# chenhonghua/MVIP-NeRF

Measured on NVIDIA B200. Metric: rays/sec (train fwd+bwd, 64+64 samples), higher is better.
Workload: dtype bf16

## Files before the change

mvip_nerf_b200/csrc/mlp_backward.cu:

```cuda
#include "mlp_pair.cuh"
#include <stdlib.h>

namespace {
using namespace mlp;

constexpr int kCSteps = 9;

struct ChainParams {
  const uint8_t* packed;
  const float4* d_raw;
  const uint8_t* stash;
  uint8_t* dz;
  int64_t n_points;
  int64_t n_tiles;
  uint32_t* flags;
  uint32_t* cons_stamp;
  uint32_t* next_pair;
  uint32_t* credit;
  int throttle_units;
  int throttle_cycles;
  int throttle_gain;
  int stagger;
};
constexpr int kFlagsPerTile = 10;

__device__ __forceinline__ int chain_nchunks(int s) { return s == 0 ? 2 : 4; }

constexpr int kStagePts = 64;
constexpr int kSubStages = kTile / kStagePts;
constexpr uint32_t kHalf = kStagePts * 128;
constexpr int kNumItems = 11;
constexpr size_t kPartialSlotBytes = (size_t)256 * 320 * sizeof(float);
constexpr int kFusedSlots = 80;

#ifndef MVIP_PROF_CLUSTER
#define MVIP_PROF_CLUSTER 0
#endif
__device__ unsigned long long g_wprof[8];
__device__ unsigned long long g_lag[80][4];
__device__ __forceinline__ uint32_t globaltimer_lo() {
  uint32_t t;
  asm volatile("mov.u32 %0, %%globaltimer_lo;" : "=r"(t));
  return t;
}
#ifdef MVIP_TRACE_BWD
__device__ long long g_btrace[20][12];
#define BTR(hs, ev) do { if (tr_on) g_btrace[hs][ev] = clock64(); } while (0)
#else
#define BTR(hs, ev)
#endif

struct WItem {
  int a_chunk;
  int m_blocks;
  int nb;
  int b_chunk[5];
  int dst;
  int ld;
  int col[5];
  int valid[5];
  int bias;
  int cost;
};

__constant__ WItem kItems[kNumItems] = {
    {kDzHidden, 1, 5, {33, 34, 35, 36, 37}, kPViewsW, 283, {0, 64, 128, 192, 256}, {64, 64, 64, 64, 27}, kPViewsB, 7},
    {kDzFeat, 2, 4, {29, 30, 31, 32, 0}, kPFeatW, 256, {0, 64, 128, 192, 0}, {64, 64, 64, 64, 0}, kPFeatB, 8},
    {kDzTrunk + 0, 2, 4, {25, 26, 27, 28, 0}, 14, 256, {0, 64, 128, 192, 0}, {64, 64, 64, 64, 0}, 15, 8},
    {kDzTrunk + 4, 2, 4, {21, 22, 23, 24, 0}, 12, 256, {0, 64, 128, 192, 0}, {64, 64, 64, 64, 0}, 13, 8},
    {kDzTrunk + 8, 2, 4, {17, 18, 19, 20, 0}, 10, 319, {63, 127, 191, 255, 0}, {64, 64, 64, 64, 0}, 11, 8},
    {kDzTrunk + 8, 2, 1, {0, 0, 0, 0, 0}, 10, 319, {0, 0, 0, 0, 0}, {63, 0, 0, 0, 0}, -1, 5},
    {kDzTrunk + 12, 2, 4, {13, 14, 15, 16, 0}, 8, 256, {0, 64, 128, 192, 0}, {64, 64, 64, 64, 0}, 9, 8},
    {kDzTrunk + 16, 2, 4, {9, 10, 11, 12, 0}, 6, 256, {0, 64, 128, 192, 0}, {64, 64, 64, 64, 0}, 7, 8},
    {kDzTrunk + 20, 2, 4, {5, 6, 7, 8, 0}, 4, 256, {0, 64, 128, 192, 0}, {64, 64, 64, 64, 0}, 5, 8},
    {kDzTrunk + 24, 2, 4, {1, 2, 3, 4, 0}, 2, 256, {0, 64, 128, 192, 0}, {64, 64, 64, 64, 0}, 3, 8},
    {kDzTrunk + 28, 2, 1, {0, 0, 0, 0, 0}, 0, 63, {0, 0, 0, 0, 0}, {63, 0, 0, 0, 0}, 1, 5},
};
constexpr int kRealItems = kNumItems;

struct Segment {
  int item;
  int t0, t1;
  int stride;
};

struct WParams {
  const uint8_t* stash;
  const uint8_t* dz;
  int64_t n_tiles;
  float* partials;
  float* bias_partials;
  Segment* segs;
};

constexpr int kFThreads = 512;
constexpr int kFSlots = 8, kFLag = 2;
constexpr int kFStages = (4 * 64) / kStagePts;
constexpr uint32_t kFStageBytes = 4 * kHalf;
constexpr uint32_t kFSmemW = 0;
constexpr uint32_t kFSmemStg = kFSmemW + kFSlots * kSlotBytes2;
constexpr uint32_t kFSmemWg = kFSmemStg + 2 * kActChunk;
constexpr uint32_t kFSmemBytes = kFSmemWg + kFStages * kFStageBytes;
struct FItem {
  int slot_item;
  int flag;
  int a_src, b_src;
  int a_chunk[2][2];
  int b_chunk[2][2];
  int n_b, n_mma;
  int transposed;
  int ld, col0, n_cols;
  int drain_ranks;
  int bias_ranks;
  int zero_lo, zero_hi;
  int cost;
};
constexpr int kFusedItems = 12;
#ifndef MVIP_SMALL_COST
#define MVIP_SMALL_COST 10
#endif
#define MVIP_FULL_ITEM(it, fl, a0, b0) {it, fl, 0, 1, {{a0, a0 + 1}, {a0 + 2, a0 + 3}}, {{b0, b0 + 1}, {b0 + 2, b0 + 3}}, 2, 256, 0, 256, 0, 256, 3, 3, 0, 0, 10}
__constant__ FItem kFItems[kFusedItems] = {
    MVIP_FULL_ITEM(1, 1, kDzFeat, 29),
    MVIP_FULL_ITEM(2, 2, kDzTrunk + 0, 25),
    MVIP_FULL_ITEM(3, 3, kDzTrunk + 4, 21),
    MVIP_FULL_ITEM(4, 4, kDzTrunk + 8, 17),
    MVIP_FULL_ITEM(6, 5, kDzTrunk + 12, 13),
    MVIP_FULL_ITEM(7, 6, kDzTrunk + 16, 9),
    MVIP_FULL_ITEM(8, 7, kDzTrunk + 20, 5),
    MVIP_FULL_ITEM(9, 8, kDzTrunk + 24, 1),
    {5, 4, 0, 1, {{kDzTrunk + 8, kDzTrunk + 9}, {kDzTrunk + 10, kDzTrunk + 11}}, {{0, 0}, {0, 0}}, 1, 128, 0, 64, 0, 64, 3, 0, 0, 0, MVIP_SMALL_COST},
    {10, 9, 0, 1, {{kDzTrunk + 28, kDzTrunk + 29}, {kDzTrunk + 30, kDzTrunk + 31}}, {{0, 0}, {0, 0}}, 1, 128, 0, 64, 0, 64, 3, 3, 0, 0, MVIP_SMALL_COST},
    {0, 0, 1, 0, {{33, 34}, {35, 36}}, {{kDzHidden, 0}, {kDzHidden + 1, 0}}, 1, 128, 1, 320, 0, 128, 3, 0, 256, 320, MVIP_SMALL_COST},
    {0, 0, 0, 1, {{kDzHidden, kDzHidden + 1}, {kDzHidden, kDzHidden + 1}}, {{37, 0}, {37, 0}}, 1, 128, 0, 320, 256, 64, 1, 1, 0, 256, MVIP_SMALL_COST},
};
struct FusedPlan {
  unsigned char item[kFusedSlots], k[kFusedSlots], n[kFusedSlots];
};


__global__ void __cluster_dims__(2, 1, 1) __launch_bounds__(kFThreads, 1)
backward_fused_kernel(const ChainParams p, const WParams wp, const FusedPlan plan) {
  constexpr int kG = kGroupBars2;
  extern __shared__ uint8_t smem_raw[];
  uint8_t* smem = reinterpret_cast<uint8_t*>((reinterpret_cast<uintptr_t>(smem_raw) + 1023) & ~uintptr_t(1023));
  __shared__ uint64_t bar_gfull[kG], bar_gempty[kG], bar_acc, bar_act, bar_hi;
  __shared__ uint64_t bar_wfull[kFStages], bar_wempty[kFStages], bar_wacc;
  __shared__ uint64_t bar_sfull[2], bar_sfree[2];
  __shared__ uint32_t tmem_base_s;
  __shared__ uint32_t it_q[4];
  __shared__ uint64_t bar_it[4];
  __shared__ uint32_t w_ready_s;
  volatile uint32_t* w_ready = &w_ready_s;

  const int tid = threadIdx.x, warp = tid >> 5, lane = tid & 31;
  const uint32_t rank = cluster_ctarank();
  const int cluster = blockIdx.x >> 1, n_clusters = gridDim.x >> 1;
  const int64_t n_pairs = (p.n_tiles + 1) / 2;
  const uint8_t* wT = p.packed + kFwdBytes;

  const int wj = plan.item[cluster], wk = plan.k[cluster], wn = plan.n[cluster];
  const FItem& fit = kFItems[wj];
  const bool w_active = wk < p.n_tiles;
  auto watch_flags = [&]() {
    if (!w_active) return;
    const int n_my = ((int)p.n_tiles - wk + wn - 1) / wn;
    unsigned long long l_sum = 0, l_max = 0;
    int ready = 0;
    while (ready < n_my) {
      const int idx = ready + lane;
      uint32_t stamp = 0;
      if (idx < n_my) stamp = ld_acquire_gpu(p.flags + (size_t)(wk + idx * wn) * kFlagsPerTile + fit.flag);
      const uint32_t got = __ballot_sync(0xffffffffu, stamp != 0u);
      const int prefix = (got == 0xffffffffu) ? 32 : __ffs(~got) - 1;
      if (prefix > 0) {
        if (lane < prefix) { const uint32_t lag = globaltimer_lo() - (stamp & ~1u); l_sum += lag; l_max = lag > l_max ? lag : l_max; }
        ready += prefix;
        __threadfence_block();
        if (lane == 0) *w_ready = (uint32_t)ready;
      } else {
        __nanosleep(100);
      }
    }
    for (int o = 16; o > 0; o >>= 1) {
      l_sum += __shfl_xor_sync(0xffffffffu, l_sum, o);
      const unsigned long long m = __shfl_xor_sync(0xffffffffu, l_max, o);
      l_max = m > l_max ? m : l_max;
    }
    if (rank == 0 && lane == 0) { g_lag[cluster][0] = l_sum; g_lag[cluster][1] = l_max; }
  };

  if (tid == 0) {
    for (int i = 0; i < kG; ++i) {
      mbar_init(&bar_gfull[i], rank == 0 ? 2 : 1);
      mbar_init(&bar_gempty[i], 1);
    }
    mbar_init(&bar_acc, 1); mbar_init(&bar_act, 16); mbar_init(&bar_hi, 16);
    for (int i = 0; i < kFStages; ++i) {
      mbar_init(&bar_wfull[i], rank == 0 ? 2 : 1);
      mbar_init(&bar_wempty[i], 1 + 2);
    }
    mbar_init(&bar_wacc, 1);
    for (int i = 0; i < 4; ++i) mbar_init(&bar_it[i], 1);
    it_q[0] = (uint32_t)cluster;
    w_ready_s = 0;
    for (int i = 0; i < 2; ++i) { mbar_init(&bar_sfull[i], 8); mbar_init(&bar_sfree[i], 1); }
    mbar_fence_init();
    mbar_arrive(&bar_it[0]);
    if (rank == 0) {
      Segment sg;
      sg.item = w_active ? fit.slot_item : -1; sg.t0 = wk; sg.t1 = w_active ? (int)p.n_tiles : wk; sg.stride = wn;
      wp.segs[cluster] = sg;
    }
  }
  if (warp == 9) tmem_alloc_2cta(&tmem_base_s, 512);
  tc_fence_before();
  __syncthreads();
  cluster_sync_all();
  tc_fence_after();
  const uint32_t tmem_base = tmem_base_s;
  auto get_it = [&](uint32_t k) -> int64_t {
    mbar_wait(&bar_it[k & 3u], (k >> 2) & 1u);
    return (int64_t)reinterpret_cast<volatile uint32_t*>(it_q)[k & 3u];
  };

  if (warp < 8) {
    const int q = warp & 3, ch = warp >> 2;
    const int r = q * 32 + lane;
    const uint32_t lane_base = (uint32_t)(q * 32) << 16;
    const uint32_t tA = tmem_base + lane_base;
    const uint32_t tD = tA + 128 + ch * 64;
    const float* small = reinterpret_cast<const float*>(p.packed + kSmallOff);
    const uint32_t stg_row = smem_u32(smem + kFSmemStg + ch * kActChunk + q * 4096) + (uint32_t)(lane >> 3) * 1024u + (uint32_t)(lane & 7) * 128u;
    const uint32_t stg_x7 = (uint32_t)(lane & 7) << 4;
    uint32_t acc_phase = 0, so_n = 0;
    auto act_arrive = [&]() {
      __syncwarp();
      if (lane == 0) {
        if (rank == 0) mbar_arrive(&bar_act);
        else mbar_arrive_cluster(mapa_u32(smem_u32(&bar_act), 0));
      }
    };
    auto hi_arrive = [&]() {
      __syncwarp();
      if (lane == 0) {
        if (rank == 0) mbar_arrive(&bar_hi);
        else mbar_arrive_cluster(mapa_u32(smem_u32(&bar_hi), 0));
      }
    };

    if (p.stagger > 0) {
      const long long t0 = clock64(), delay = (long long)cluster * p.stagger;
      while (clock64() - t0 < delay) __nanosleep(200);
    }
    for (uint32_t kq = 0;; ++kq) {
      const int64_t it = get_it(kq);
      if (it >= n_pairs) break;
      uint32_t nxt = 0;
      if (warp == 0 && lane == 0 && rank == 0) nxt = (uint32_t)n_clusters + atom_add_relaxed_gpu(p.next_pair, 1u);
      const int64_t tile = 2 * it + (int64_t)rank;
      const bool tile_valid = tile < p.n_tiles;
      const int64_t g = tile * kTile + r;
      const bool valid = tile_valid && g < p.n_points;
      const uint32_t* masks = reinterpret_cast<const uint32_t*>(p.stash + (size_t)(tile_valid ? tile : 0) * kStashTileBytes + kStashMaskOff);
#ifdef MVIP_TRACE_BWD
      const bool tr_on = cluster == 0 && rank == 0 && warp == 0 && lane == 0 && kq == 3;
      int tr_hs = 0;
#endif

      auto stage_out = [&](const uint32_t (&pk)[32]) {
        const uint32_t sb = so_n & 1u;
        if (so_n > 0) mbar_wait(&bar_sfree[sb ^ 1u], ((so_n - 1) >> 1) & 1u);
        ++so_n;
        BTR(tr_hs, 7);
#pragma unroll
        for (int gq = 0; gq < 8; ++gq)
          sts128(stg_row | (((uint32_t)gq << 4) ^ stg_x7), pk[4 * gq], pk[4 * gq + 1], pk[4 * gq + 2], pk[4 * gq + 3]);
        BTR(tr_hs, 8);
        fence_proxy_async_smem();
        __syncwarp();
        BTR(tr_hs, 9);
        if (lane == 0) mbar_arrive(&bar_sfull[sb]);
        BTR(tr_hs, 10);
      };
      auto load_mask = [&](int s, int h) -> uint2 {
        if (!valid) return make_uint2(0u, 0u);
        if (s < 1) return make_uint2(~0u, ~0u);
        return __ldg(reinterpret_cast<const uint2*>(masks + mask_word_index(8 - s, r, h, ch)));
      };

      uint32_t pk[32];
      const float4 dr = valid ? __ldg(p.d_raw + g) : make_float4(0.f, 0.f, 0.f, 0.f);
      {
        const uint2 mw = valid ? __ldg(reinterpret_cast<const uint2*>(masks + mask_word_index(8, r, 0, ch))) : make_uint2(0u, 0u);
#pragma unroll
        for (int b = 0; b < 4; ++b) {
          const int c0 = ch * 64 + 16 * b;
          float v[16];
#pragma unroll
          for (int j4 = 0; j4 < 4; ++j4) {
            const float4 w0 = __ldg(reinterpret_cast<const float4*>(small + kSmWRgb + c0 + 4 * j4));
            const float4 w1 = __ldg(reinterpret_cast<const float4*>(small + kSmWRgb + 128 + c0 + 4 * j4));
            const float4 w2 = __ldg(reinterpret_cast<const float4*>(small + kSmWRgb + 256 + c0 + 4 * j4));
            v[4 * j4 + 0] = dr.x * w0.x + dr.y * w1.x + dr.z * w2.x;
            v[4 * j4 + 1] = dr.x * w0.y + dr.y * w1.y + dr.z * w2.y;
            v[4 * j4 + 2] = dr.x * w0.z + dr.y * w1.z + dr.z * w2.z;
            v[4 * j4 + 3] = dr.x * w0.w + dr.y * w1.w + dr.z * w2.w;
          }
          const uint32_t m = (b < 2 ? mw.x : mw.y) >> (8 * (b & 1));
#pragma unroll
          for (int i = 0; i < 8; ++i) pk[8 * b + i] = mask_bf16x2(pack_bf16x2(v[2 * i], v[2 * i + 1]), (m >> i) & 0x00010001u);
        }
        tmem_st32(tA + ch * 32, pk);
        tmem_st_wait();
        tc_fence_before();
        act_arrive();
        stage_out(pk);
      }

      uint2 mw_next = load_mask(0, 0);
#pragma unroll 1
      for (int s = 0; s < kCSteps; ++s) {
        if (warp == 0 && lane == 0 && ((rank == 0 && s == 4) || (rank == 1 && s == 6))) {
          uint32_t* slot = p.next_pair + 16 + 4 * cluster + ((kq + 1) & 3u);
          if (rank == 0) {
            if (nxt > 0xFFFFFu) nxt = 0xFFFFFu;
            st_relaxed_gpu(slot, ((kq + 1) << 20) | nxt);
          } else {
            uint32_t v = ld_relaxed_gpu(slot);
            const long long t0 = clock64();
            while ((v >> 20) != ((kq + 1) & 0xFFFu)) {
              if (clock64() - t0 > 8000000000LL) { printf("mvip: fused backward tile hand-out timeout cluster %d\n", cluster); __trap(); }
              v = ld_relaxed_gpu(slot);
            }
            nxt = v & 0xFFFFFu;
          }
          reinterpret_cast<volatile uint32_t*>(it_q)[(kq + 1) & 3u] = nxt;
          mbar_arrive(&bar_it[(kq + 1) & 3u]);
        }
#pragma unroll 1
        for (int h = 0; h < 2; ++h) {
          const uint2 mw = mw_next;
          mw_next = (h == 0) ? load_mask(s, 1) : load_mask(s + 1 < kCSteps ? s + 1 : 0, 0);
          {
            uint32_t raw[4][16];
            BTR(tr_hs, 0);
            mbar_wait(&bar_acc, acc_phase);
            BTR(tr_hs, 1);
            acc_phase ^= 1;
            tc_fence_after();
            if (h == 1 && s < kCSteps - 1) tmem_st32(tA + ch * 32, pk);
            load_half(tD, raw);
            if (h == 1 && s < kCSteps - 1) tmem_st_wait();
            BTR(tr_hs, 2);
            tc_fence_before();
            if (h == 0 || s < kCSteps - 1) act_arrive();
            BTR(tr_hs, 3);
#pragma unroll
            for (int b = 0; b < 4; ++b) {
              float v[16];
              if (s == 1) {
                const int c0 = h * 128 + ch * 64 + 16 * b;
#pragma unroll
                for (int j4 = 0; j4 < 4; ++j4) {
                  const float4 w = __ldg(reinterpret_cast<const float4*>(small + kSmWAlpha + c0 + 4 * j4));
                  v[4 * j4 + 0] = __uint_as_float(raw[b][4 * j4 + 0]) + dr.w * w.x;
                  v[4 * j4 + 1] = __uint_as_float(raw[b][4 * j4 + 1]) + dr.w * w.y;
                  v[4 * j4 + 2] = __uint_as_float(raw[b][4 * j4 + 2]) + dr.w * w.z;
                  v[4 * j4 + 3] = __uint_as_float(raw[b][4 * j4 + 3]) + dr.w * w.w;
                }
              } else {
#pragma unroll
                for (int j = 0; j < 16; ++j) v[j] = __uint_as_float(raw[b][j]);
              }
              const uint32_t m = (b < 2 ? mw.x : mw.y) >> (8 * (b & 1));
#pragma unroll
              for (int i = 0; i < 8; ++i) pk[8 * b + i] = mask_bf16x2(pack_bf16x2(v[2 * i], v[2 * i + 1]), (m >> i) & 0x00010001u);
            }
          }
          BTR(tr_hs, 4);
          if (h == 1 && s < kCSteps - 1) {
            tmem_st32(tA + 64 + ch * 32, pk);
            tmem_st_wait();
            tc_fence_before();
            hi_arrive();
          }
          BTR(tr_hs, 5);
          stage_out(pk);
          BTR(tr_hs, 6);
#ifdef MVIP_TRACE_BWD
          ++tr_hs;
#endif
        }
      }
    }
    if (warp < 4 && w_active) {
      mbar_wait(&bar_wacc, 0);
      tc_fence_after();
      float* part = wp.partials + (size_t)cluster * (kPartialSlotBytes / sizeof(float));
      if ((fit.drain_ranks >> rank) & 1) {
        for (int c0 = 0; c0 < fit.n_cols; c0 += 32) {
          uint32_t acc[32];
          tmem_ld32(tmem_base + lane_base + 256 + c0, acc);
          tmem_ld_wait();
          if (fit.transposed) {
#pragma unroll
            for (int j = 0; j < 32; ++j) part[(size_t)(c0 + j) * fit.ld + 128 * rank + r] = __uint_as_float(acc[j]);
          } else {
            float* prow = part + (size_t)(128 * rank + r) * fit.ld + fit.col0 + c0;
#pragma unroll
            for (int j = 0; j < 32; j += 4)
              *reinterpret_cast<float4*>(prow + j) = make_float4(__uint_as_float(acc[j]), __uint_as_float(acc[j + 1]),
                                                                 __uint_as_float(acc[j + 2]), __uint_as_float(acc[j + 3]));
          }
        }
      }
      if (fit.zero_hi > fit.zero_lo) {
        const int row = 64 * (int)rank + (r & 63), half = r >> 6, w = (fit.zero_hi - fit.zero_lo) / 2;
        float* z = part + (size_t)row * fit.ld + fit.zero_lo + half * w;
        for (int j = 0; j < w; j += 4) *reinterpret_cast<float4*>(z + j) = make_float4(0.f, 0.f, 0.f, 0.f);
      }
    }
  } else if (warp == 8) {
    if (lane == 0) {
      uint32_t j = 0; int slot = 0;
      for (uint32_t kq = 0; get_it(kq) < n_pairs; ++kq) {
        int cbase = 0;
        for (int s = 0; s < kCSteps; ++s) {
          const int n = chain_nchunks(s);
          for (int h = 0; h < 2; ++h, ++j) {
            if (j >= (uint32_t)kFLag) mbar_wait(&bar_gempty[(j - kFLag) % kG], ((j - kFLag) / kG) & 1u);
            uint64_t* full = &bar_gfull[j % kG];
            mbar_arrive_expect_tx(full, (uint32_t)n * kSlotBytes2);
            for (int ci = 0; ci < n; ++ci) {
              const uint8_t* src = wT + (size_t)(cbase + ci) * kW256 + (size_t)(2 * h + (int)rank) * kSlotBytes2;
              tma_load_1d(smem + kFSmemW + slot * kSlotBytes2, src, kSlotBytes2, full);
              if (++slot == kFSlots) slot = 0;
            }
          }
          cbase += n;
        }
      }
    }
  } else if (warp == 9) {
    if (rank == 1 && lane == 0) {
      uint32_t j = 0;
      for (uint32_t kq = 0; get_it(kq) < n_pairs; ++kq) {
        for (int c = 0; c < 2 * kCSteps; ++c, ++j) {
          mbar_wait(&bar_gfull[j % kG], (j / kG) & 1u);
          mbar_arrive_cluster(mapa_u32(smem_u32(&bar_gfull[j % kG]), 0));
        }
      }
    } else if (rank == 0) {
      watch_flags();
    }
  } else if (warp == 10) {
    if (rank == 0) {
      uint32_t act_phase = 0, hi_phase = 0, j = 0;
      long long c_t0 = clock64(), c_act = 0, c_full = 0, c_x = 0;
      const uint32_t idesc = umma_idesc_bf16(256, 128, 0, 0);
      const uint32_t tA = tmem_base;
      const uint32_t tDm = tA + 128;
      const uint32_t w_lo = desc_lo2(smem_u32(smem) + kFSmemW);
      const uint32_t w_end = w_lo + kFSlots * (kSlotBytes2 >> 4);
      uint32_t bpos = w_lo;
      auto next_slot = [&](uint32_t b) { b += (kSlotBytes2 >> 4); return b == w_end ? w_lo : b; };
      for (uint32_t kq = 0; get_it(kq) < n_pairs; ++kq) {
#pragma unroll 1
        for (int s = 0; s < kCSteps; ++s) {
#pragma unroll 1
          for (int h = 0; h < 2; ++h, ++j) {
            const uint32_t b1 = bpos, b2 = next_slot(b1), b3 = next_slot(b2), b4 = next_slot(b3);
            bpos = (s == 0) ? b3 : next_slot(b4);
            uint64_t* gempty = &bar_gempty[j % kG];
            c_x = clock64();
            mbar_wait(&bar_gfull[j % kG], (j / kG) & 1u);
            c_full += clock64() - c_x; c_x = clock64();
            mbar_wait(&bar_act, act_phase);
            c_act += clock64() - c_x;
            act_phase ^= 1;
            tc_fence_after();
            if (elect_one_sync()) {
#pragma unroll
              for (int kk = 0; kk < 4; ++kk) mma2_ts(tDm, tA + kk * 8, b1 + kk * 2, idesc, kk > 0 ? 1u : 0u);
#pragma unroll
              for (int kk = 0; kk < 4; ++kk) mma2_ts(tDm, tA + 32 + kk * 8, b2 + kk * 2, idesc, 1u);
              if (s == 0) {
                umma_commit_2cta(gempty, 3);
                umma_commit_2cta(&bar_acc, 3);
              }
            }
            __syncwarp();
            if (s > 0) {
              if (h == 0) {
                c_x = clock64();
                mbar_wait(&bar_hi, hi_phase);
                c_act += clock64() - c_x;
                hi_phase ^= 1;
                tc_fence_after();
              }
              if (elect_one_sync()) {
#pragma unroll
                for (int kk = 0; kk < 4; ++kk) mma2_ts(tDm, tA + 64 + kk * 8, b3 + kk * 2, idesc, 1u);
#pragma unroll
                for (int kk = 0; kk < 4; ++kk) mma2_ts(tDm, tA + 96 + kk * 8, b4 + kk * 2, idesc, 1u);
                umma_commit_2cta(gempty, 3);
                umma_commit_2cta(&bar_acc, 3);
              }
              __syncwarp();
            }
          }
        }
      }
      if (cluster == MVIP_PROF_CLUSTER && lane == 0) { g_wprof[0] = clock64() - c_t0; g_wprof[1] = c_act; g_wprof[2] = c_full; }
    } else {
      watch_flags();
    }
  } else if (warp == 11) {
    if (w_active) {
      const uint64_t pol = l2_policy_evict_first();
      const int n_loads = 2 + fit.n_b;
      const uint32_t stage_tx = (uint32_t)n_loads * kHalf;
      const bool loader = lane < n_loads;
      const int lj = lane < 2 ? lane : lane - 2;
      const bool from_stash = loader && (lane < 2 ? fit.a_src : fit.b_src);
      const int my_chunk = loader ? (lane < 2 ? fit.a_chunk[rank][lj] : fit.b_chunk[rank][lj]) : 0;
      const int n_my = ((int)p.n_tiles - wk + wn - 1) / wn;
      int stage = 0; uint32_t phase = 0;
      long long p_flag = 0, p_empty = 0, p_t0 = clock64();
      unsigned long long l_ready = 0;
      uint32_t fenced = 0;
      if (from_stash) {
        tma_prefetch_l2(wp.stash + (size_t)wk * kStashTileBytes + (size_t)my_chunk * kActChunk, kActChunk);
        if (n_my > 1) tma_prefetch_l2(wp.stash + (size_t)(wk + wn) * kStashTileBytes + (size_t)my_chunk * kActChunk, kActChunk);
      }
      for (int i = 0; i < n_my; ++i) {
        const int t = wk + i * wn;
        const uint8_t* src = (from_stash ? wp.stash + (size_t)t * kStashTileBytes : wp.dz + (size_t)t * kDzTileBytes) + (size_t)my_chunk * kActChunk;
        if (from_stash && i + 2 < n_my) tma_prefetch_l2(src + (size_t)2 * wn * kStashTileBytes, kActChunk);
        {
          long long t0 = clock64();
          if ((uint32_t)i >= fenced) {
            uint32_t r = *w_ready;
            if (r > (uint32_t)i) ++l_ready;
            while (r <= (uint32_t)i) {
              if (clock64() - t0 > 8000000000LL) { if (lane == 0) printf("mvip: fused wgrad flag timeout cluster %d tile %d flag %d\n", cluster, t, fit.flag); __trap(); }
              r = *w_ready;
            }
            fence_proxy_async_global();
            fenced = r;
          } else {
            ++l_ready;
          }
          p_flag += clock64() - t0;
          if (rank == 0 && lane == 0) {
            p.cons_stamp[(size_t)t * kFlagsPerTile + fit.flag] = globaltimer_lo();
            red_add_relaxed_gpu(p.credit + 1, (fit.flag == 0 || fit.flag == 4) ? 1u : 2u);
          }
        }
        for (int h = 0; h < kSubStages; ++h) {
          uint8_t* sbase = smem + kFSmemWg + stage * kFStageBytes;
          long long te = clock64();
          mbar_wait(&bar_wempty[stage], phase ^ 1);
          p_empty += clock64() - te;
          if (lane == 0) mbar_arrive_expect_tx(&bar_wfull[stage], stage_tx);
          __syncwarp();
          if (loader) tma_load_1d_hint(sbase + lane * kHalf, src + h * kHalf, kHalf, &bar_wfull[stage], pol);
          if (++stage == kFStages) { stage = 0; phase ^= 1; }
        }
      }
      if (cluster == MVIP_PROF_CLUSTER && rank == 0 && lane == 0) { g_wprof[5] = p_flag; g_wprof[6] = p_empty; g_wprof[7] = clock64() - p_t0; }
      if (rank == 0 && lane == 0) { g_lag[cluster][2] = n_my; g_lag[cluster][3] = l_ready; }
    }
  } else if (warp == 12) {
    if (w_active) {
      int stage = 0; uint32_t phase = 0;
      if (rank == 0) {
        const uint32_t idesc = umma_idesc_bf16(256, fit.n_mma, 1, 1);
        const uint32_t d0 = tmem_base + 256;
        bool first = true;
        long long w_t0 = clock64(), w_full = 0;
        for (int t = wk; t < p.n_tiles; t += wn) {
          for (int h = 0; h < kSubStages; ++h) {
            const uint32_t sbase = smem_u32(smem) + kFSmemWg + stage * kFStageBytes;
            const uint32_t a_lo = desc_lo_mn(sbase, kHalf), b_lo = desc_lo_mn(sbase + 2 * kHalf, kHalf);
            long long tw = clock64();
            mbar_wait(&bar_wfull[stage], phase);
            w_full += clock64() - tw;
            tc_fence_after();
            if (elect_one_sync()) {
#pragma unroll
              for (int ks = 0; ks < kStagePts / 16; ++ks) {
                const uint32_t ko = (uint32_t)ks * (2048u >> 4);
                mma2_ss(d0, a_lo + ko, b_lo + ko, idesc, (first && ks == 0) ? 0u : 1u);
              }
              umma_commit_2cta(&bar_wempty[stage], 3);
            }
            __syncwarp();
            first = false;
            if (++stage == kFStages) { stage = 0; phase ^= 1; }
          }
        }
        if (elect_one_sync()) umma_commit_2cta(&bar_wacc, 3);
        __syncwarp();
        if (cluster == MVIP_PROF_CLUSTER && lane == 0) { g_wprof[3] = clock64() - w_t0; g_wprof[4] = w_full; }
      } else if (lane == 0) {
        for (int t = wk; t < p.n_tiles; t += wn) {
          for (int h = 0; h < kSubStages; ++h) {
            mbar_wait(&bar_wfull[stage], phase);
            mbar_arrive_cluster(mapa_u32(smem_u32(&bar_wfull[stage]), 0));
            if (++stage == kFStages) { stage = 0; phase ^= 1; }
          }
        }
      }
    }
  } else if ((warp == 13 || warp == 14) && w_active) {
    static_assert(kStagePts == 64, "the bias warps assume 64-point stages");
    const int t4 = (warp - 13) * 32 + lane;
    const int fg = t4 & 15, rg = t4 >> 4;
    const uint32_t boff = (uint32_t)(fg >> 3) * kHalf + (uint32_t)rg * 16u * 128u;
    const uint32_t g7 = (uint32_t)(fg & 7);
    float acc[8] = {0.f, 0.f, 0.f, 0.f, 0.f, 0.f, 0.f, 0.f};
    const bool do_bias = (fit.bias_ranks >> rank) & 1;
    int stage = 0; uint32_t phase = 0;
    for (int t = wk; t < p.n_tiles; t += wn) {
      for (int h = 0; h < kSubStages; ++h) {
        mbar_wait(&bar_wfull[stage], phase);
        if (do_bias) {
          const uint32_t a32 = smem_u32(smem) + kFSmemWg + stage * kFStageBytes + boff;
#pragma unroll
          for (int i = 0; i < 16; ++i) {
            uint32_t w0, w1, w2, w3;
            asm volatile("ld.shared.v4.u32 {%0, %1, %2, %3}, [%4];" : "=r"(w0), "=r"(w1), "=r"(w2), "=r"(w3)
                         : "r"(a32 + (uint32_t)i * 128u + ((g7 ^ (uint32_t)(i & 7)) << 4)));
            acc[0] += __uint_as_float(w0 << 16); acc[1] += __uint_as_float(w0 & 0xffff0000u);
            acc[2] += __uint_as_float(w1 << 16); acc[3] += __uint_as_float(w1 & 0xffff0000u);
            acc[4] += __uint_as_float(w2 << 16); acc[5] += __uint_as_float(w2 & 0xffff0000u);
            acc[6] += __uint_as_float(w3 << 16); acc[7] += __uint_as_float(w3 & 0xffff0000u);
          }
        }
        __syncwarp();
        if (lane == 0) mbar_arrive(&bar_wempty[stage]);
        if (++stage == kFStages) { stage = 0; phase ^= 1; }
      }
    }
#pragma unroll
    for (int e = 0; e < 8; ++e) acc[e] += __shfl_xor_sync(0xffffffffu, acc[e], 16);
    if (lane < 16) {
      float* bias_out = wp.bias_partials + (size_t)cluster * 512 + (size_t)(warp - 13) * 256 + 128 * rank + 8 * fg;
#pragma unroll
      for (int e = 0; e < 8; ++e) bias_out[e] = acc[e];
    }
  } else if (warp == 15) {
    if (lane == 0) {
      uint32_t n = 0;
      uint32_t* pend[2] = {nullptr, nullptr};
      auto publish = [&](uint32_t*& f) {
        if (f) { fence_proxy_async_global(); st_release_gpu(f, globaltimer_lo() | 1u); red_add_relaxed_gpu(p.credit, 2u); f = nullptr; }
      };
      for (uint32_t kq = 0;; ++kq) {
        const int64_t it = get_it(kq);
        if (it >= n_pairs) break;
        const int64_t tile = 2 * it + (int64_t)rank;
        const bool tile_valid = tile < p.n_tiles;
        uint8_t* dz_tile = p.dz + (size_t)(tile_valid ? tile : 0) * kDzTileBytes;
        uint32_t* tile_flags = p.flags + (size_t)(tile_valid ? tile : 0) * kFlagsPerTile;
        for (int c = 0; c < 1 + 2 * kCSteps; ++c, ++n) {
          const int s = (c - 1) >> 1, h = (c - 1) & 1;
          const int chunk = (c == 0) ? kDzHidden : ((s == 0 ? kDzFeat : kDzTrunk + 4 * (s - 1)) + 2 * h);
          const uint32_t sb = n & 1u;
          if (c == 0 && p.throttle_cycles > 0) {
            const long long t0 = clock64();
            if (p.throttle_gain > 0) {
              const int excess = (int)(ld_relaxed_gpu(p.credit) - ld_relaxed_gpu(p.credit + 1)) / 2 - p.throttle_units;
              long long delay = (long long)excess * p.throttle_gain;
              if (delay > p.throttle_cycles) delay = p.throttle_cycles;
              while (clock64() - t0 < delay) __nanosleep(200);
            } else {
              while ((int)(ld_relaxed_gpu(p.credit) - ld_relaxed_gpu(p.credit + 1)) > 2 * p.throttle_units && clock64() - t0 < p.throttle_cycles) __nanosleep(500);
            }
          }
          mbar_wait(&bar_sfull[sb], (n >> 1) & 1u);
          if (tile_valid) tma_store_1d(dz_tile + (size_t)chunk * kActChunk, smem + kFSmemStg, 2 * kActChunk);
          tma_store_commit();
          tma_store_wait_read0();
          mbar_arrive(&bar_sfree[sb]);
          tma_store_wait_all2();
          publish(pend[1]);
          pend[1] = pend[0];
          pend[0] = (tile_valid && (c == 0 || h == 1)) ? tile_flags + (c == 0 ? 0 : 1 + s) : nullptr;
        }
      }
      tma_store_wait_all0();
      publish(pend[1]);
      publish(pend[0]);
    }
  }

  tc_fence_before();
  __syncthreads();
  cluster_sync_all();
  if (warp == 9) tmem_dealloc_2cta(tmem_base, 512);
}

constexpr int kHeadFloats = 256 + 4 + 384 + 4;
constexpr int kHeadMaxBlocks = 1184;
constexpr int kHgRows = 64;
constexpr int kHgStages = 4;
constexpr uint32_t kHgPiece = kHgRows * 128;
constexpr uint32_t kHgStageBytes = 6 * kHgPiece + kHgRows * 16;
constexpr int kHgThreads = 288;
constexpr size_t kHgSmemBytes = (size_t)kHgStages * kHgStageBytes + 1024;

__device__ __forceinline__ void unpack_bf16x8(const uint4 v, float (&f)[8]) {
  f[0] = __uint_as_float(v.x << 16); f[1] = __uint_as_float(v.x & 0xffff0000u);
  f[2] = __uint_as_float(v.y << 16); f[3] = __uint_as_float(v.y & 0xffff0000u);
  f[4] = __uint_as_float(v.z << 16); f[5] = __uint_as_float(v.z & 0xffff0000u);
  f[6] = __uint_as_float(v.w << 16); f[7] = __uint_as_float(v.w & 0xffff0000u);
}

__global__ void __launch_bounds__(kHgThreads, 1) head_grads_kernel(const float4* __restrict__ d_raw, const uint8_t* __restrict__ stash,
                                                                int64_t n_points, int64_t n_half, float* __restrict__ out) {
  extern __shared__ uint8_t hg_smem_raw[];
  __shared__ float red[8][kHeadFloats];
  __shared__ uint64_t full[kHgStages], empty[kHgStages];
  uint8_t* ring = reinterpret_cast<uint8_t*>((reinterpret_cast<uintptr_t>(hg_smem_raw) + 1023) & ~(uintptr_t)1023);
  const int tid = threadIdx.x, warp = tid >> 5, lane = tid & 31;
  if (tid == 0) {
    for (int s = 0; s < kHgStages; ++s) { mbar_init(&full[s], 1); mbar_init(&empty[s], 8); }
    mbar_fence_init();
  }
  __syncthreads();
  if (warp == 8) {
    const uint64_t pol = l2_policy_evict_first();
    int it = 0;
    for (int64_t h = blockIdx.x; h < n_half; h += gridDim.x, ++it) {
      const int s = it % kHgStages;
      if (it >= kHgStages) mbar_wait(&empty[s], ((it / kHgStages) & 1) ^ 1);
      uint8_t* dst = ring + (size_t)s * kHgStageBytes;
      const uint8_t* tile = stash + (size_t)(h >> 1) * kStashTileBytes + (size_t)(h & 1) * kHgPiece;
      const int64_t left = n_points - h * kHgRows;
      const uint32_t d_bytes = (uint32_t)(left < kHgRows ? left : kHgRows) * 16u;
      if (lane == 0) mbar_arrive_expect_tx(&full[s], 6 * kHgPiece + d_bytes);
      __syncwarp();
      if (lane < 4) tma_load_1d_hint(dst + lane * kHgPiece, tile + (size_t)(kStashH + 28 + lane) * kActChunk, kHgPiece, &full[s], pol);
      else if (lane < 6) tma_load_1d_hint(dst + lane * kHgPiece, tile + (size_t)(kStashHidden + lane - 4) * kActChunk, kHgPiece, &full[s], pol);
      else if (lane == 6) tma_load_1d(dst + 6 * kHgPiece, d_raw + h * kHgRows, d_bytes, &full[s]);
    }
  } else {
    float aa[8] = {0, 0, 0, 0, 0, 0, 0, 0};
    float ar[8] = {0, 0, 0, 0, 0, 0, 0, 0}, ag[8] = {0, 0, 0, 0, 0, 0, 0, 0}, ab[8] = {0, 0, 0, 0, 0, 0, 0, 0};
    float4 ds = make_float4(0.f, 0.f, 0.f, 0.f);
    const uint32_t h8_piece = (uint32_t)(lane >> 3) * kHgPiece, hid_piece = (uint32_t)(4 + ((lane & 15) >> 3)) * kHgPiece;
    const int g8 = lane & 7, par = lane >> 4;
    int it = 0;
    for (int64_t h = blockIdx.x; h < n_half; h += gridDim.x, ++it) {
      const int s = it % kHgStages;
      mbar_wait(&full[s], (it / kHgStages) & 1);
      const uint8_t* st = ring + (size_t)s * kHgStageBytes;
      const float4* dsm = reinterpret_cast<const float4*>(st + 6 * kHgPiece);
      const int64_t left = n_points - h * kHgRows;
      const int valid = (int)(left < kHgRows ? left : kHgRows);
#pragma unroll
      for (int i = 0; i < 8; ++i) {
        const int row = warp * 8 + i;
        const float4 d = row < valid ? dsm[row] : make_float4(0.f, 0.f, 0.f, 0.f);
        float f[8];
        unpack_bf16x8(*reinterpret_cast<const uint4*>(st + h8_piece + chunk_off16(row, g8)), f);
#pragma unroll
        for (int e = 0; e < 8; ++e) aa[e] += d.w * f[e];
        ds.x += d.x; ds.y += d.y; ds.z += d.z; ds.w += d.w;
      }
#pragma unroll
      for (int i = 0; i < 4; ++i) {
        const int row = warp * 8 + 2 * i + par;
        const float4 d = row < valid ? dsm[row] : make_float4(0.f, 0.f, 0.f, 0.f);
        float f[8];
        unpack_bf16x8(*reinterpret_cast<const uint4*>(st + hid_piece + chunk_off16(row, g8)), f);
#pragma unroll
        for (int e = 0; e < 8; ++e) { ar[e] += d.x * f[e]; ag[e] += d.y * f[e]; ab[e] += d.z * f[e]; }
      }
      __syncwarp();
      if (lane == 0) mbar_arrive(&empty[s]);
    }
#pragma unroll
    for (int e = 0; e < 8; ++e) {
      ar[e] += __shfl_xor_sync(FULL_MASK, ar[e], 16);
      ag[e] += __shfl_xor_sync(FULL_MASK, ag[e], 16);
      ab[e] += __shfl_xor_sync(FULL_MASK, ab[e], 16);
      red[warp][lane * 8 + e] = aa[e];
      if (lane < 16) {
        red[warp][260 + lane * 8 + e] = ar[e];
        red[warp][260 + 128 + lane * 8 + e] = ag[e];
        red[warp][260 + 256 + lane * 8 + e] = ab[e];
      }
    }
    if (lane == 31) { red[warp][256] = ds.w; red[warp][644] = ds.x; red[warp][645] = ds.y; red[warp][646] = ds.z; }
    if (lane == 30) { red[warp][257] = red[warp][258] = red[warp][259] = 0.f; red[warp][647] = 0.f; }
  }
  __syncthreads();
  float* o = out + (size_t)blockIdx.x * kHeadFloats;
  for (int e = tid; e < kHeadFloats; e += kHgThreads) {
    float s = 0.f;
#pragma unroll
    for (int k = 0; k < 8; ++k) s += red[k][e];
    o[e] = s;
  }
}

struct ReduceParams {
// ... 278 lines not shown
```

mvip_nerf_b200/csrc/mlp_pack.cu:

```cuda
#include "mlp_common.cuh"

namespace {
using namespace mlp;

struct Src {
  int param;
  int rows;
  int base;
  int stride_n;
  int stride_k;
  int valid_k;
};

__device__ __forceinline__ Src fwd_src(int c) {
  if (c == 0) return {kPW(0), 256, 0, 63, 1, 63};
  if (c <= 16) return {kPW(1 + (c - 1) / 4), 256, 64 * ((c - 1) % 4), 256, 1, 64};
  if (c == 17) return {kPW(5), 256, 0, 319, 1, 63};
  if (c <= 21) return {kPW(5), 256, 63 + 64 * (c - 18), 319, 1, 64};
  if (c <= 29) return {kPW(6 + (c - 22) / 4), 256, 64 * ((c - 22) % 4), 256, 1, 64};
  if (c <= 33) return {kPFeatW, 256, 64 * (c - 30), 256, 1, 64};
  if (c <= 37) return {kPViewsW, 128, 64 * (c - 34), 283, 1, 64};
  return {kPViewsW, 128, 256, 283, 1, 27};
}
__device__ __forceinline__ Src bwd_src(int c) {
  if (c <= 1) return {kPViewsW, 256, 64 * c * 283, 1, 283, 64};
  if (c <= 5) return {kPFeatW, 256, 64 * (c - 2) * 256, 1, 256, 64};
  int layer = 7 - (c - 6) / 4, j = (c - 6) % 4;
  int ld = (layer == 5) ? 319 : 256;
  return {kPW(layer), 256, 64 * j * ld + ((layer == 5) ? 63 : 0), 1, ld, 64};
}

__global__ void pack_kernel(ParamPtrs pp, uint8_t* __restrict__ packed) {
  const int total_groups = (int)((kFwdBytes + kBwdBytes) / 16);
  for (int gidx = blockIdx.x * blockDim.x + threadIdx.x; gidx < total_groups; gidx += gridDim.x * blockDim.x) {
    size_t byte = (size_t)gidx * 16;
    Src s;
    size_t chunk_base;
    uint32_t in_chunk;
    if (byte < kFwdBytes) {
      int c = byte < 34 * (size_t)kW256 ? (int)(byte / kW256) : 34 + (int)((byte - 34 * (size_t)kW256) / kW128);
      s = fwd_src(c);
      chunk_base = fwd_chunk_off(c);
      in_chunk = (uint32_t)(byte - chunk_base);
    } else {
      size_t b2 = byte - kFwdBytes;
      int c = (int)(b2 / kW256);
      s = bwd_src(c);
      chunk_base = kFwdBytes + (size_t)c * kW256;
      in_chunk = (uint32_t)(b2 - (size_t)c * kW256);
    }
    uint32_t n = (in_chunk >> 10) * 8 + ((in_chunk >> 7) & 7);
    uint32_t g = ((in_chunk >> 4) & 7) ^ (n & 7);
    const float* src = pp.p[s.param] + s.base + (size_t)n * s.stride_n;
    float v[8];
#pragma unroll
    for (int e = 0; e < 8; ++e) {
      int k = g * 8 + e;
      v[e] = (k < s.valid_k) ? __ldg(src + (size_t)k * s.stride_k) : 0.f;
    }
    uint4 o = make_uint4(pack_bf16x2(v[0], v[1]), pack_bf16x2(v[2], v[3]), pack_bf16x2(v[4], v[5]), pack_bf16x2(v[6], v[7]));
    *reinterpret_cast<uint4*>(packed + chunk_base + in_chunk) = o;
  }
  float* sm = reinterpret_cast<float*>(packed + kSmallOff);
  for (int i = blockIdx.x * blockDim.x + threadIdx.x; i < kSmallFloats; i += gridDim.x * blockDim.x) {
    float v = 0.f;
    if (i < kSmBiasFeat) v = pp.p[2 * (i / 256) + 1][i % 256];
    else if (i < kSmBiasViews) v = pp.p[kPFeatB][i - kSmBiasFeat];
    else if (i < kSmWAlpha) v = pp.p[kPViewsB][i - kSmBiasViews];
    else if (i < kSmBAlpha) v = pp.p[kPAlphaW][i - kSmWAlpha];
    else if (i == kSmBAlpha) v = pp.p[kPAlphaB][0];
    else if (i >= kSmWRgb && i < kSmBRgb) v = pp.p[kPRgbW][i - kSmWRgb];
    else if (i >= kSmBRgb && i < kSmBRgb + 3) v = pp.p[kPRgbB][i - kSmBRgb];
    sm[i] = v;
  }
}

}

extern "C" {

size_t mvip_mlp_packed_bytes(void) { return mlp::kPackedBytes; }

int mvip_mlp_pack_weights(const float* const* params, void* packed, void* stream) {
  MVIP_REQUIRE(params && packed, MVIP_E_INVALID, "mvip_mlp_pack_weights: null pointer");
  MVIP_REQUIRE(mvip_aligned(packed, 1024), MVIP_E_INVALID, "mvip_mlp_pack_weights: packed must be 1024-byte aligned");
  mlp::ParamPtrs pp;
  for (int i = 0; i < MVIP_MLP_NUM_PARAMS; ++i) {
    MVIP_REQUIRE(params[i], MVIP_E_INVALID, "mvip_mlp_pack_weights: params[%d] is null", i);
    pp.p[i] = params[i];
  }
  pack_kernel<<<mvip_num_sms() * 2, 256, 0, (cudaStream_t)stream>>>(pp, static_cast<uint8_t*>(packed));
  MVIP_LAUNCH_OK("pack_kernel");
  return MVIP_OK;
}

}
```

Before: 1.251 million.

## Prefetch next tile inputs and pre-issue its first activation during last step

In the fused backward chain, the first-layer input activation for the next tile (d_raw times the RGB weights, masked) is now computed and stored to tensor memory during the final step of the current tile, so the MMA issuer can start the next tile sooner. Two steps earlier, the next tile's d_raw row and mask words are prefetched into L2. The aim is to hide the tile-boundary bubble where the MMA pipeline waits on this input. In exchange the code adds extra get_it waits and duplicated work: the next tile still recomputes the same pk via input_pk before staging it out. The interleaving with the act_arrive barrier protocol also becomes more delicate.

```diff
diff --git a/mvip_nerf_b200/csrc/mlp_backward.cu b/mvip_nerf_b200/csrc/mlp_backward.cu
--- a/mvip_nerf_b200/csrc/mlp_backward.cu
+++ b/mvip_nerf_b200/csrc/mlp_backward.cu
@@ -234,6 +234,35 @@
     const uint32_t stg_row = smem_u32(smem + kFSmemStg + ch * kActChunk + q * 4096) + (uint32_t)(lane >> 3) * 1024u + (uint32_t)(lane & 7) * 128u;
     const uint32_t stg_x7 = (uint32_t)(lane & 7) << 4;
     uint32_t acc_phase = 0, so_n = 0;
+    auto input_pk = [&](const float4 d, const uint2 mw, uint32_t (&pk)[32]) {
+#pragma unroll
+      for (int b = 0; b < 4; ++b) {
+        const int c0 = ch * 64 + 16 * b;
+        float v[16];
+#pragma unroll
+        for (int j4 = 0; j4 < 4; ++j4) {
+          const float4 w0 = __ldg(reinterpret_cast<const float4*>(small + kSmWRgb + c0 + 4 * j4));
+          const float4 w1 = __ldg(reinterpret_cast<const float4*>(small + kSmWRgb + 128 + c0 + 4 * j4));
+          const float4 w2 = __ldg(reinterpret_cast<const float4*>(small + kSmWRgb + 256 + c0 + 4 * j4));
+          v[4 * j4 + 0] = d.x * w0.x + d.y * w1.x + d.z * w2.x;
+          v[4 * j4 + 1] = d.x * w0.y + d.y * w1.y + d.z * w2.y;
+          v[4 * j4 + 2] = d.x * w0.z + d.y * w1.z + d.z * w2.z;
+          v[4 * j4 + 3] = d.x * w0.w + d.y * w1.w + d.z * w2.w;
+        }
+        const uint32_t m = (b < 2 ? mw.x : mw.y) >> (8 * (b & 1));
+#pragma unroll
+        for (int i = 0; i < 8; ++i) pk[8 * b + i] = mask_bf16x2(pack_bf16x2(v[2 * i], v[2 * i + 1]), (m >> i) & 0x00010001u);
+      }
+    };
+    auto next_input = [&](uint32_t kq, const float4*& d, const uint2*& m) -> bool {
+      const int64_t itn = get_it(kq + 1);
+      const int64_t tile_n = 2 * itn + (int64_t)rank, g_n = tile_n * kTile + r;
+      const bool ok = itn < n_pairs && tile_n < p.n_tiles && g_n < p.n_points;
+      d = p.d_raw + (ok ? g_n : 0);
+      m = reinterpret_cast<const uint2*>(p.stash + (size_t)(ok ? tile_n : 0) * kStashTileBytes + kStashMaskOff) + mask_word_index(8, r, 0, ch) / 2;
+      return ok;
+    };
+    bool pre = false;
     auto act_arrive = [&]() {
       __syncwarp();
       if (lane == 0) {
@@ -293,28 +322,14 @@
       const float4 dr = valid ? __ldg(p.d_raw + g) : make_float4(0.f, 0.f, 0.f, 0.f);
       {
         const uint2 mw = valid ? __ldg(reinterpret_cast<const uint2*>(masks + mask_word_index(8, r, 0, ch))) : make_uint2(0u, 0u);
-#pragma unroll
-        for (int b = 0; b < 4; ++b) {
-          const int c0 = ch * 64 + 16 * b;
-          float v[16];
-#pragma unroll
-          for (int j4 = 0; j4 < 4; ++j4) {
-            const float4 w0 = __ldg(reinterpret_cast<const float4*>(small + kSmWRgb + c0 + 4 * j4));
-            const float4 w1 = __ldg(reinterpret_cast<const float4*>(small + kSmWRgb + 128 + c0 + 4 * j4));
-            const float4 w2 = __ldg(reinterpret_cast<const float4*>(small + kSmWRgb + 256 + c0 + 4 * j4));
-            v[4 * j4 + 0] = dr.x * w0.x + dr.y * w1.x + dr.z * w2.x;
-            v[4 * j4 + 1] = dr.x * w0.y + dr.y * w1.y + dr.z * w2.y;
-            v[4 * j4 + 2] = dr.x * w0.z + dr.y * w1.z + dr.z * w2.z;
-            v[4 * j4 + 3] = dr.x * w0.w + dr.y * w1.w + dr.z * w2.w;
-          }
-          const uint32_t m = (b < 2 ? mw.x : mw.y) >> (8 * (b & 1));
-#pragma unroll
-          for (int i = 0; i < 8; ++i) pk[8 * b + i] = mask_bf16x2(pack_bf16x2(v[2 * i], v[2 * i + 1]), (m >> i) & 0x00010001u);
-        }
-        tmem_st32(tA + ch * 32, pk);
-        tmem_st_wait();
-        tc_fence_before();
-        act_arrive();
+        input_pk(dr, mw, pk);
+        if (!pre) {
+          tmem_st32(tA + ch * 32, pk);
+          tmem_st_wait();
+          tc_fence_before();
+          act_arrive();
+        }
+        pre = false;
         stage_out(pk);
       }
 
@@ -337,6 +352,13 @@
           }
           reinterpret_cast<volatile uint32_t*>(it_q)[(kq + 1) & 3u] = nxt;
           mbar_arrive(&bar_it[(kq + 1) & 3u]);
+        }
+        if (s == kCSteps - 2) {
+          const float4* d; const uint2* m;
+          if (next_input(kq, d, m)) {
+            asm volatile("prefetch.global.L2 [%0];" ::"l"(d));
+            asm volatile("prefetch.global.L2 [%0];" ::"l"(m));
+          }
         }
 #pragma unroll 1
         for (int h = 0; h < 2; ++h) {
@@ -355,6 +377,16 @@
             BTR(tr_hs, 2);
             tc_fence_before();
             if (h == 0 || s < kCSteps - 1) act_arrive();
+            if (h == 1 && s == kCSteps - 1 && get_it(kq + 1) < n_pairs) {
+              const float4* d; const uint2* m;
+              const bool ok = next_input(kq, d, m);
+              input_pk(ok ? __ldg(d) : make_float4(0.f, 0.f, 0.f, 0.f), ok ? __ldg(m) : make_uint2(0u, 0u), pk);
+              tmem_st32(tA + ch * 32, pk);
+              tmem_st_wait();
+              tc_fence_before();
+              act_arrive();
+              pre = true;
+            }
             BTR(tr_hs, 3);
 #pragma unroll
             for (int b = 0; b < 4; ++b) {
```

New measurement: 1.162 million, median of 6. -7.1%, worse.

## Split backward UMMA into per-channel N=64 halves with per-channel accumulator barriers

Applied to the files above, without the earlier changes.

The backward chain MMA, previously one N=128 UMMA per group, is split into two N=64 halves, one per epilogue channel. Each half commits its own accumulator barrier, so each channel's epilogue warps can start draining TMEM as soon as their half is done. The second half-step now waits on per-channel drain barriers plus a final barrier, and the weight packing permutes backward N rows so each half reads a contiguous quarter slot. This aims to overlap tensor-core work with the epilogue, at the cost of twice as many MMA instructions, commits and barrier waits, and a more intricate phase protocol.

```diff
diff --git a/mvip_nerf_b200/csrc/mlp_backward.cu b/mvip_nerf_b200/csrc/mlp_backward.cu
--- a/mvip_nerf_b200/csrc/mlp_backward.cu
+++ b/mvip_nerf_b200/csrc/mlp_backward.cu
@@ -144,7 +144,7 @@
   constexpr int kG = kGroupBars2;
   extern __shared__ uint8_t smem_raw[];
   uint8_t* smem = reinterpret_cast<uint8_t*>((reinterpret_cast<uintptr_t>(smem_raw) + 1023) & ~uintptr_t(1023));
-  __shared__ uint64_t bar_gfull[kG], bar_gempty[kG], bar_acc, bar_act, bar_hi;
+  __shared__ uint64_t bar_gfull[kG], bar_gempty[kG], bar_acc[2], bar_fin, bar_dr[2], bar_act, bar_hi;
   __shared__ uint64_t bar_wfull[kFStages], bar_wempty[kFStages], bar_wacc;
   __shared__ uint64_t bar_sfull[2], bar_sfree[2];
   __shared__ uint32_t tmem_base_s;
@@ -195,7 +195,8 @@
       mbar_init(&bar_gfull[i], rank == 0 ? 2 : 1);
       mbar_init(&bar_gempty[i], 1);
     }
-    mbar_init(&bar_acc, 1); mbar_init(&bar_act, 16); mbar_init(&bar_hi, 16);
+    for (int c = 0; c < 2; ++c) { mbar_init(&bar_acc[c], 1); mbar_init(&bar_dr[c], 8); }
+    mbar_init(&bar_fin, 1); mbar_init(&bar_act, 16); mbar_init(&bar_hi, 16);
     for (int i = 0; i < kFStages; ++i) {
       mbar_init(&bar_wfull[i], rank == 0 ? 2 : 1);
       mbar_init(&bar_wempty[i], 1 + 2);
@@ -233,7 +234,14 @@
     const float* small = reinterpret_cast<const float*>(p.packed + kSmallOff);
     const uint32_t stg_row = smem_u32(smem + kFSmemStg + ch * kActChunk + q * 4096) + (uint32_t)(lane >> 3) * 1024u + (uint32_t)(lane & 7) * 128u;
     const uint32_t stg_x7 = (uint32_t)(lane & 7) << 4;
-    uint32_t acc_phase = 0, so_n = 0;
+    uint32_t acc_phase = 0, fin_phase = 0, so_n = 0;
+    auto dr_arrive = [&]() {
+      __syncwarp();
+      if (lane == 0) {
+        if (rank == 0) mbar_arrive(&bar_dr[ch]);
+        else mbar_arrive_cluster(mapa_u32(smem_u32(&bar_dr[ch]), 0));
+      }
+    };
     auto act_arrive = [&]() {
       __syncwarp();
       if (lane == 0) {
@@ -345,16 +353,21 @@
           {
             uint32_t raw[4][16];
             BTR(tr_hs, 0);
-            mbar_wait(&bar_acc, acc_phase);
+            mbar_wait(&bar_acc[ch], acc_phase);
+            acc_phase ^= 1;
+            if (h == 1) {
+              mbar_wait(&bar_fin, fin_phase);
+              fin_phase ^= 1;
+            }
             BTR(tr_hs, 1);
-            acc_phase ^= 1;
             tc_fence_after();
             if (h == 1 && s < kCSteps - 1) tmem_st32(tA + ch * 32, pk);
             load_half(tD, raw);
             if (h == 1 && s < kCSteps - 1) tmem_st_wait();
             BTR(tr_hs, 2);
             tc_fence_before();
-            if (h == 0 || s < kCSteps - 1) act_arrive();
+            if (h == 0) dr_arrive();
+            else if (s < kCSteps - 1) act_arrive();
             BTR(tr_hs, 3);
 #pragma unroll
             for (int b = 0; b < 4; ++b) {
@@ -456,15 +469,15 @@
     }
   } else if (warp == 10) {
     if (rank == 0) {
-      uint32_t act_phase = 0, hi_phase = 0, j = 0;
+      uint32_t act_phase = 0, hi_phase = 0, dr_phase = 0, j = 0;
       long long c_t0 = clock64(), c_act = 0, c_full = 0, c_x = 0;
-      const uint32_t idesc = umma_idesc_bf16(256, 128, 0, 0);
       const uint32_t tA = tmem_base;
-      const uint32_t tDm = tA + 128;
       const uint32_t w_lo = desc_lo2(smem_u32(smem) + kFSmemW);
       const uint32_t w_end = w_lo + kFSlots * (kSlotBytes2 >> 4);
       uint32_t bpos = w_lo;
       auto next_slot = [&](uint32_t b) { b += (kSlotBytes2 >> 4); return b == w_end ? w_lo : b; };
+      constexpr uint32_t kQuarterB = (32 * 128) >> 4;
+      const uint32_t idesc_q = umma_idesc_bf16(256, 64, 0, 0);
       for (uint32_t kq = 0; get_it(kq) < n_pairs; ++kq) {
 #pragma unroll 1
         for (int s = 0; s < kCSteps; ++s) {
@@ -472,40 +485,52 @@
           for (int h = 0; h < 2; ++h, ++j) {
             const uint32_t b1 = bpos, b2 = next_slot(b1), b3 = next_slot(b2), b4 = next_slot(b3);
             bpos = (s == 0) ? b3 : next_slot(b4);
-            uint64_t* gempty = &bar_gempty[j % kG];
             c_x = clock64();
             mbar_wait(&bar_gfull[j % kG], (j / kG) & 1u);
             c_full += clock64() - c_x; c_x = clock64();
-            mbar_wait(&bar_act, act_phase);
+            if (h == 0) {
+              mbar_wait(&bar_act, act_phase);
+              act_phase ^= 1;
+            }
             c_act += clock64() - c_x;
-            act_phase ^= 1;
             tc_fence_after();
-            if (elect_one_sync()) {
-#pragma unroll
-              for (int kk = 0; kk < 4; ++kk) mma2_ts(tDm, tA + kk * 8, b1 + kk * 2, idesc, kk > 0 ? 1u : 0u);
-#pragma unroll
-              for (int kk = 0; kk < 4; ++kk) mma2_ts(tDm, tA + 32 + kk * 8, b2 + kk * 2, idesc, 1u);
-              if (s == 0) {
-                umma_commit_2cta(gempty, 3);
-                umma_commit_2cta(&bar_acc, 3);
-              }
-            }
-            __syncwarp();
-            if (s > 0) {
-              if (h == 0) {
+#pragma unroll 1
+            for (int c = 0; c < 2; ++c) {
+              const uint32_t tDq = tA + 128 + 64 * c, bq = (uint32_t)c * kQuarterB;
+              if (h == 1) {
                 c_x = clock64();
-                mbar_wait(&bar_hi, hi_phase);
+                mbar_wait(&bar_dr[c], dr_phase);
+                if (c == 1) dr_phase ^= 1;
                 c_act += clock64() - c_x;
-                hi_phase ^= 1;
                 tc_fence_after();
               }
               if (elect_one_sync()) {
 #pragma unroll
-                for (int kk = 0; kk < 4; ++kk) mma2_ts(tDm, tA + 64 + kk * 8, b3 + kk * 2, idesc, 1u);
-#pragma unroll
-                for (int kk = 0; kk < 4; ++kk) mma2_ts(tDm, tA + 96 + kk * 8, b4 + kk * 2, idesc, 1u);
-                umma_commit_2cta(gempty, 3);
-                umma_commit_2cta(&bar_acc, 3);
+                for (int kk = 0; kk < 4; ++kk) mma2_ts(tDq, tA + kk * 8, b1 + bq + kk * 2, idesc_q, kk > 0 ? 1u : 0u);
+#pragma unroll
+                for (int kk = 0; kk < 4; ++kk) mma2_ts(tDq, tA + 32 + kk * 8, b2 + bq + kk * 2, idesc_q, 1u);
+              }
+              __syncwarp();
+              if (s > 0) {
+                if (h == 0 && c == 0) {
+                  c_x = clock64();
+                  mbar_wait(&bar_hi, hi_phase);
+                  c_act += clock64() - c_x;
+                  hi_phase ^= 1;
+                  tc_fence_after();
+                }
+                if (elect_one_sync()) {
+#pragma unroll
+                  for (int kk = 0; kk < 4; ++kk) mma2_ts(tDq, tA + 64 + kk * 8, b3 + bq + kk * 2, idesc_q, 1u);
+#pragma unroll
+                  for (int kk = 0; kk < 4; ++kk) mma2_ts(tDq, tA + 96 + kk * 8, b4 + bq + kk * 2, idesc_q, 1u);
+                }
+                __syncwarp();
+              }
+              if (elect_one_sync()) {
+                if (c == 1) umma_commit_2cta(&bar_gempty[j % kG], 3);
+                umma_commit_2cta(&bar_acc[c], 3);
+                if (h == 1 && c == 1) umma_commit_2cta(&bar_fin, 3);
               }
               __syncwarp();
             }
diff --git a/mvip_nerf_b200/csrc/mlp_pack.cu b/mvip_nerf_b200/csrc/mlp_pack.cu
--- a/mvip_nerf_b200/csrc/mlp_pack.cu
+++ b/mvip_nerf_b200/csrc/mlp_pack.cu
@@ -51,7 +51,8 @@
     }
     uint32_t n = (in_chunk >> 10) * 8 + ((in_chunk >> 7) & 7);
     uint32_t g = ((in_chunk >> 4) & 7) ^ (n & 7);
-    const float* src = pp.p[s.param] + s.base + (size_t)n * s.stride_n;
+    const uint32_t nf = byte < kFwdBytes ? n : (n & ~0x60u) | ((n & 0x20u) << 1) | ((n & 0x40u) >> 1);
+    const float* src = pp.p[s.param] + s.base + (size_t)nf * s.stride_n;
     float v[8];
 #pragma unroll
     for (int e = 0; e < 8; ++e) {
```

New measurement: 1.269 million before, 1.213 million after, median of 6. 4.4% lower.
